# bjing2016/mdgen

Hardware: AMD Instinct MI355X
Metric: sampled MD frames/sec (higher is better)
Workload: dtype bf16; 1 GPU; tetrapeptide_fwdsim_crop4_T1000_B16; batch_per_gpu=16, num_frames=1000, crop=4, euler_steps=49, hipgraph=True, parallelism=batch-sharded x1, no collective

## Files before the change

### mdgen_amd/csrc/k_flash.hip

```cpp
#include "kernels.h"
#include "panel.h"
#include <type_traits>

namespace mdg {

__device__ __forceinline__ bf16x8 frag16(const unsigned char* p) { return *reinterpret_cast<const bf16x8*>(p); }

__device__ __forceinline__ bf16x8 frag8(const unsigned char* p) {
    const u32x2 v = *reinterpret_cast<const u32x2*>(p);
    const u32x4 w = u32x4{v[0], v[1], 0u, 0u};
    return __builtin_bit_cast(bf16x8, w);
}

struct KTile {
    u32x4 k0;
    u32x4 k1;
};
__device__ __forceinline__ void k_consts(KTile& t) {
    t.k1 = u32x4{0u, 0u, 0x3f803f80u, 0u};
    asm volatile("" : "+v"(t.k1));
}
struct VTile {
    u32x4 v0;
    u32x4 v1;
// ... 60 lines not shown
    float e[16];
#pragma unroll
    for (int j = 0; j < 16; ++j) e[j] = __builtin_amdgcn_exp2f(s[j]);
#pragma unroll
    for (int j = 0; j < 4; ++j) {
        pc.p0[j] = pack_bf16(e[2 * j], e[2 * j + 1]);
        pc.p1[j] = pack_bf16(e[8 + 2 * j], e[9 + 2 * j]);
    }
#pragma unroll
    for (int g = 0; g < 4; ++g) {
        __builtin_amdgcn_sched_group_barrier(0x008, 1, 0);
        __builtin_amdgcn_sched_group_barrier(0x402, 6, 0);
    }
    asm volatile("" : "+v"(pc.p0), "+v"(pc.p1) : "v"(k0), "v"(k1), "v"(qn.q0), "v"(qn.q1));
}

constexpr float kDefer = 8.f;

__device__ __forceinline__ void softmax_stats(Half& st, f32x16& s, QTile& q, uint32_t vm, int hh) {
    if (vm != 0xffffffffu) mask_scores(s, vm, hh);
    float t = fmaxf(s[0], s[1]);
#pragma unroll
    for (int r = 2; r < 16; r += 2) t = fmaxf(fmaxf(t, s[r]), s[r + 1]);
    t = half_max(t);
    if ((__builtin_amdgcn_ballot_w64(t > kDefer) | st.unanch) != 0) {
        const bool fin = t > -1e29f;
        const bool un = (st.unanch >> lane_id()) & 1ull;
        const bool mv = (t > kDefer) | (un & fin & (t < -kDefer));
        st.unanch &= ~__builtin_amdgcn_ballot_w64(fin);
        const float r = set_shift(q, mv ? st.m + t : st.m, hh);
        const float e = r - st.m;
        st.m = r;
        const float a = __builtin_amdgcn_exp2f(fminf(-e, 0.f));
#pragma unroll
        for (int i = 0; i < 16; ++i) {
            st.o[i] *= a;
            s[i] -= e;
        }
    }
}

#ifdef MDGEN_DEV_FLASH_STAMPS
__device__ unsigned long long g_flash_stamps[32768 * 16];
extern "C" int mdgen_dev_flash_stamps(void* host, size_t bytes) {
    return (int)hipMemcpyFromSymbol(host, HIP_SYMBOL(g_flash_stamps), bytes);
}
#define FLASH_STAMP(slot, v)                                                                          \
    if (lane == 0 && (long)blockIdx.x * 4 + w < 32768) g_flash_stamps[((long)blockIdx.x * 4 + w) * 16 + (slot)] = (v)
__device__ unsigned long long g_fproj_stamps[8192 * 16];
extern "C" int mdgen_dev_fproj_stamps(void* host, size_t bytes) {
    return (int)hipMemcpyFromSymbol(host, HIP_SYMBOL(g_fproj_stamps), bytes);
}
#define FPROJ_STAMP(slot, v)                                                                          \
    if (lane_id() == 0 && (long)blockIdx.x * 4 + w < 8192) g_fproj_stamps[((long)blockIdx.x * 4 + w) * 16 + (slot)] = (v)
#define FLASH_STAMP_ROW(w, hg) ((w) + 4096 * (hg))
#else
#define FLASH_STAMP(slot, v)
#define FPROJ_STAMP(slot, v)
#define FLASH_STAMP_ROW(w, hg) (w)
#endif

template <int N, class F>
__device__ __forceinline__ void static_for(F&& f) {
    if constexpr (N > 0) {
        static_for<N - 1>(f);
        f(std::integral_constant<int, N - 1>{});
    }
}

struct FlashStoreGlobal {
    __bf16* obuf;
    AxisMap ax;
    int seq, head;
    __device__ __forceinline__ void row(int, int pos, u32x2 a, u32x2 b, u32x2 c) const {
        u32x2* d = reinterpret_cast<u32x2*>(obuf + ax.token(seq, pos) * kC + head * kDH + (lane_id() >> 5) * 12);
        d[0] = a;
        d[1] = b;
        d[2] = c;
    }
    __device__ __forceinline__ void pad(int, int) const {}
};

template <int NQ>
struct FlashPre {
    QTile q[NQ];
    u32x4 kb0;
    u32x2 kb1;
    f32x4 bvl[3];
    u32x4 k0t0;
    u32x2 k0t1;
    uint32_t vmw;
};

__device__ __forceinline__ void* flash_uniform_ptr(const unsigned char* q_) {
    const unsigned long long a = (unsigned long long)q_;
    const unsigned lo = __builtin_amdgcn_readfirstlane((unsigned)a), hi = __builtin_amdgcn_readfirstlane((unsigned)(a >> 32));
    return (void*)(((unsigned long long)hi << 32) | lo);
}

template <int NQ>
__device__ __forceinline__ void flash_prefetch(const FlashParams p, const int seq, const int head, const int qc, FlashPre<NQ>& pre) {
    const int lane = lane_id(), hh = lane >> 5;
    const int len = p.ax.len, nt = p.ax.ntile();
    const long ftile = (long)(seq * kH + head) * nt;
    const unsigned char* qb = p.qf + ftile * kFragQ;
    const int qt0 = NQ * qc;
#pragma unroll
    for (int j = 0; j < NQ; ++j) {
        const int qt = (qt0 + j) * 32 < len ? qt0 + j : qt0;
        pre.q[j].q0 = frag16(qb + (long)qt * kFragQ + lane * 16);
        pre.q[j].q1 = frag8(qb + (long)qt * kFragQ + 1024 + lane * 8);
    }
    const bool bias_alone = (len & 31) == 0 && len >= 32;
    const unsigned char* kb = p.kf + (ftile + (bias_alone ? (len >> 5) : 0)) * kFragK;
    pre.kb0 = *reinterpret_cast<const u32x4*>(kb + hh * 32 * 16);
    pre.kb1 = *reinterpret_cast<const u32x2*>(kb + 1024 + hh * 32 * 8);
    const f32x4* bv = reinterpret_cast<const f32x4*>(p.bias_v + head * kDH + hh * 12);
    pre.bvl[0] = bv[0];
    pre.bvl[1] = bv[1];
    pre.bvl[2] = bv[2];
    const __amdgpu_buffer_rsrc_t krs = __builtin_amdgcn_make_buffer_rsrc(flash_uniform_ptr(p.kf + ftile * kFragK), 0, 0x7fffffff, 0x00020000);
    pre.k0t0 = __builtin_amdgcn_raw_buffer_load_b128(krs, lane * 16, 0, 0);
    pre.k0t1 = __builtin_amdgcn_raw_buffer_load_b64(krs, lane * 8 + 1024, 0, 0);
    pre.vmw = (p.vmask + (long)seq * p.vmask_stride)[lane];
}

template <int NQ, class Store>
__device__ __forceinline__ void flash_job(const FlashParams p, const int seq, const int head, const int qc, const int w,
                                          const FlashPre<NQ> pre, const Store store) {
    const int lane = lane_id(), hh = lane >> 5, ql = lane & 31;
    FLASH_STAMP(0, __builtin_amdgcn_s_memtime());
    FLASH_STAMP(4, __builtin_amdgcn_s_memrealtime());
    const int len = p.ax.len, nt = p.ax.ntile();
    const long ftile = (long)(seq * kH + head) * nt;
    const int qt0 = NQ * qc;
    QTile q[NQ];
    bool qvalid[NQ];
#pragma unroll
    for (int j = 0; j < NQ; ++j) {
        qvalid[j] = (qt0 + j) * 32 < len;
        q[j] = pre.q[j];
    }
    const bool bias_alone = (len & 31) == 0 && len >= 32;
    const u32x4 kb0 = pre.kb0;
    const u32x2 kb1 = pre.kb1;
    const f32x4 bvl[3] = {pre.bvl[0], pre.bvl[1], pre.bvl[2]};

    const __amdgpu_buffer_rsrc_t krs = __builtin_amdgcn_make_buffer_rsrc(flash_uniform_ptr(p.kf + ftile * kFragK), 0, 0x7fffffff, 0x00020000);
    const __amdgpu_buffer_rsrc_t vrs = __builtin_amdgcn_make_buffer_rsrc(flash_uniform_ptr(p.vf + ftile * kFragV), 0, 0x7fffffff, 0x00020000);
    const int koff = lane * 16, koff1 = lane * 8 + 1024;
    const int voff = ql <= kDH ? hh * 400 + ql * 16 : (int)0x80000000;
    auto issue_k = [&](KTile& t, int kt) __attribute__((always_inline)) {
        t.k0 = __builtin_amdgcn_raw_buffer_load_b128(krs, koff, kt * kFragK, 0);
        const u32x2 r = __builtin_amdgcn_raw_buffer_load_b64(krs, koff1, kt * kFragK, 0);
        t.k1[0] = r[0];
        t.k1[1] = r[1];
    };
    auto issue_v = [&](VTile& t, int kt) __attribute__((always_inline)) {
        t.v0 = __builtin_amdgcn_raw_buffer_load_b128(vrs, voff, kt * kFragV, 0);
        t.v1 = __builtin_amdgcn_raw_buffer_load_b128(vrs, voff + 800, kt * kFragV, 0);
    };
    KTile k0t;
    k0t.k0 = pre.k0t0;
    k0t.k1 = u32x4{pre.k0t1[0], pre.k0t1[1], 0x3f803f80u, 0u};
    const uint32_t* vmrow = p.vmask + (long)seq * p.vmask_stride;
    uint32_t vmw = pre.vmw;

    Half h[NQ];
    f32x16 s[2];
    PTile pt[2];
    KTile kx, ky;
    VTile vx, vy;
    int rot = 0, nrun = 1;
    auto phys = [&](int i) __attribute__((always_inline)) {
        const int t = i + rot;
        return t >= nrun ? t - nrun : t;
    };
    auto tile = [&](auto robust, int ti, KTile& kc, KTile& kn, VTile& vc, VTile& vprev) __attribute__((always_inline)) {
        constexpr bool kRobust = decltype(robust)::value;
        const int t = kRobust ? ti : phys(ti);
        const uint32_t vm = __builtin_amdgcn_readlane(vmw, t & 63);
        static_for<NQ>([&](auto J) __attribute__((always_inline)) {
            constexpr int j = decltype(J)::value;
            if constexpr (kRobust) softmax_stats(h[j], s[j & 1], q[j], vm, hh);
            else if (vm != 0xffffffffu) mask_scores(s[j & 1], vm, hh);
            __builtin_amdgcn_sched_barrier(0);
            if constexpr (j == 0) block(kc, q[1], s[1], vprev, pt[(NQ - 1) & 1], h[NQ - 1].o, s[0], pt[0]);
            else if constexpr (j < NQ - 1) block(kc, q[j + 1], s[(j + 1) & 1], vc, pt[(j - 1) & 1], h[j - 1].o, s[j & 1], pt[j & 1]);
            else block(kn, q[0], s[0], vc, pt[(j - 1) & 1], h[j - 1].o, s[j & 1], pt[j & 1]);
            __builtin_amdgcn_sched_barrier(0);
            if constexpr (j == 0) issue_v(vprev, kRobust ? ti + 1 : phys(ti + 1));
            if constexpr (j == NQ - 2) issue_k(kc, kRobust ? ti + 2 : phys(ti + 2));
            if constexpr (j == 0 || j == NQ - 2) __builtin_amdgcn_sched_barrier(0);
        });
    };
    auto run = [&](auto robust, const int nt, const int rot_) __attribute__((always_inline)) {
        rot = rot_;
        nrun = nt;
#pragma unroll
        for (int j = 0; j < NQ; ++j)
#pragma unroll
            for (int r = 0; r < 16; ++r) h[j].o[r] = opaque_zero();
        pt[(NQ - 1) & 1].p0 = pt[(NQ - 1) & 1].p1 = u32x4{0u, 0u, 0u, 0u};
        if (nt > 64) vmw = vmrow[lane];
        k_consts(kx);
        k_consts(ky);
        issue_k(kx, phys(0));
        issue_v(vy, phys(0));
        issue_k(ky, phys(1));
        issue_v(vx, phys(0));
        __builtin_amdgcn_sched_barrier(0);
        s[0] = scores(kx, q[0]);
        int t = 0;
        for (; t + 1 < nt; t += 2) {
            if ((t & 63) == 0 && t) vmw = vmrow[t + lane];
            tile(robust, t, kx, ky, vx, vy);
            tile(robust, t + 1, ky, kx, vy, vx);
        }
        const bf16x8 lp0 = __builtin_bit_cast(bf16x8, pt[(NQ - 1) & 1].p0), lp1 = __builtin_bit_cast(bf16x8, pt[(NQ - 1) & 1].p1);
        if (t < nt) {
            if ((t & 63) == 0 && t) vmw = vmrow[t + lane];
            tile(robust, t, kx, ky, vx, vy);
            h[NQ - 1].o = __builtin_amdgcn_mfma_f32_32x32x16_bf16(__builtin_bit_cast(bf16x8, vx.v0), __builtin_bit_cast(bf16x8, pt[(NQ - 1) & 1].p0), h[NQ - 1].o, 0, 0, 0);
            h[NQ - 1].o = __builtin_amdgcn_mfma_f32_32x32x16_bf16(__builtin_bit_cast(bf16x8, vx.v1), __builtin_bit_cast(bf16x8, pt[(NQ - 1) & 1].p1), h[NQ - 1].o, 0, 0, 0);
        } else {
            h[NQ - 1].o = __builtin_amdgcn_mfma_f32_32x32x16_bf16(__builtin_bit_cast(bf16x8, vy.v0), lp0, h[NQ - 1].o, 0, 0, 0);
            h[NQ - 1].o = __builtin_amdgcn_mfma_f32_32x32x16_bf16(__builtin_bit_cast(bf16x8, vy.v1), lp1, h[NQ - 1].o, 0, 0, 0);
        }
    };

    if (nt <= 64 && !p.force_robust) {
        const uint32_t want = lane == (len >> 5) ? 1u << (len & 31) : 0u;
        const bool only_bias = __builtin_amdgcn_ballot_w64(lane < nt && vmw != want) == 0;
        if (only_bias) {
            const f32x4 b0 = bvl[0], b1 = bvl[1], b2 = bvl[2];
            const u32x2 d0 = {pack_bf16(b0[0], b0[1]), pack_bf16(b0[2], b0[3])}, d1 = {pack_bf16(b1[0], b1[1]), pack_bf16(b1[2], b1[3])},
                        d2 = {pack_bf16(b2[0], b2[1]), pack_bf16(b2[2], b2[3])};
#pragma unroll
            for (int j = 0; j < NQ; ++j) {
                const int pos = (qt0 + j) * 32 + ql;
                if (qvalid[j] && pos < len) store.row(j, pos, d0, d1, d2);
                else store.pad(j, pos);
            }
            return;
        }
    }
    const int nt_fast = bias_alone ? nt - 1 : nt;
    float sbias[NQ], vbias[12];
    if (bias_alone) {
        const f32x4 b0 = bvl[0], b1 = bvl[1], b2 = bvl[2];
#pragma unroll
        for (int i = 0; i < 4; ++i) {
            vbias[i] = round_bf16(b0[i]);
            vbias[4 + i] = round_bf16(b1[i]);
            vbias[8 + i] = round_bf16(b2[i]);
        }
#pragma unroll
        for (int j = 0; j < NQ; ++j) {
            const u32x4 qa = __builtin_bit_cast(u32x4, q[j].q0);
            const u32x4 qb_ = __builtin_bit_cast(u32x4, q[j].q1);
            float d = 0.f;
#pragma unroll
            for (int i = 0; i < 4; ++i) d += bf16_lo(qa[i]) * bf16_lo(kb0[i]) + bf16_hi(qa[i]) * bf16_hi(kb0[i]);
#pragma unroll
            for (int i = 0; i < 2; ++i) d += bf16_lo(qb_[i]) * bf16_lo(kb1[i]) + bf16_hi(qb_[i]) * bf16_hi(kb1[i]);
            sbias[j] = d + __shfl_xor(d, 32, 64);
        }
    }
    bool robust_needed = p.force_robust != 0;
    {
        const uint32_t vm0 = __builtin_amdgcn_readlane(vmw, 0);
#pragma unroll
        for (int j = 0; j < NQ; ++j) {
            f32x16 s0 = scores(k0t, q[j]);
            if (vm0 != 0xffffffffu) mask_scores(s0, vm0, hh);
            float t0 = fmaxf(s0[0], s0[1]);
#pragma unroll
            for (int r = 2; r < 16; r += 2) t0 = fmaxf(fmaxf(t0, s0[r]), s0[r + 1]);
            t0 = half_max(t0);
            robust_needed |= __builtin_amdgcn_ballot_w64(!(t0 > -1e29f)) != 0;
            h[j].m = set_shift(q[j], t0 + kAnchor, hh);
        }
    }
    FLASH_STAMP(1, __builtin_amdgcn_s_memtime());
    FLASH_STAMP(6, (unsigned long long)robust_needed);
    FLASH_STAMP(8, (unsigned long long)__float_as_uint(h[0].m));
    if (!robust_needed) {
        run(std::false_type{}, nt_fast, (p.rotate && nt_fast > 2 && nt <= 64) ? (qc * nt_fast) / ((len + 32 * NQ - 1) / (32 * NQ)) : 0);
        if (bias_alone) {
#pragma unroll
            for (int j = 0; j < NQ; ++j) {
                const float pb = __builtin_amdgcn_exp2f(sbias[j] - h[j].m);
#pragma unroll
                for (int r = 0; r < 12; ++r) h[j].o[r] += pb * vbias[r];
                if (hh == 0) h[j].o[12] += pb;
            }
        }
        FLASH_STAMP(2, __builtin_amdgcn_s_memtime());
        bool bad = false;
#pragma unroll
        for (int j = 0; j < NQ; ++j) {
            const uint32_t lj = __float_as_uint(h[j].o[12]);
            bad |= (lj & 0x7f800000u) == 0x7f800000u;
            bad |= hh == 0 && (lj & 0x7f800000u) == 0u;
#pragma unroll
            for (int i = 0; i < 16; ++i) bad |= (__float_as_uint(h[j].o[i]) & 0x7f800000u) == 0x7f800000u;
        }
        FLASH_STAMP(9, (unsigned long long)__builtin_amdgcn_ballot_w64(bad));
        robust_needed = __builtin_amdgcn_ballot_w64(bad) != 0;
    }
    if (robust_needed) {
#pragma unroll
        for (int j = 0; j < NQ; ++j) {
            h[j].m = 0.f;
            h[j].unanch = ~0ull;
            set_shift(q[j], 0.f, hh);
        }
        run(std::true_type{}, nt, 0);
    }
    FLASH_STAMP(3, __builtin_amdgcn_s_memtime());
    FLASH_STAMP(11, (unsigned long long)__float_as_uint(h[0].m));
#ifdef MDGEN_DEV_FLASH_STAMPS
    if (lane == 0 && (long)blockIdx.x * 4 + w < 32768) g_flash_stamps[((long)blockIdx.x * 4 + w) * 16 + 6] |= (unsigned long long)robust_needed << 1;
#endif
#pragma unroll
    for (int j = 0; j < NQ; ++j) {
        const float l = __shfl(h[j].o[12], ql, 64);
        const int pos = (qt0 + j) * 32 + ql;
        if (qvalid[j] && pos < len) {
            const float inv = 1.0f / l;
            const f32x16 o = h[j].o;
            store.row(j, pos, u32x2{pack_bf16(o[0] * inv, o[1] * inv), pack_bf16(o[2] * inv, o[3] * inv)},
                      u32x2{pack_bf16(o[4] * inv, o[5] * inv), pack_bf16(o[6] * inv, o[7] * inv)},
                      u32x2{pack_bf16(o[8] * inv, o[9] * inv), pack_bf16(o[10] * inv, o[11] * inv)});
        } else {
            store.pad(j, pos);
        }
    }
    FLASH_STAMP(5, __builtin_amdgcn_s_memrealtime());
}

template <int NQ>
__global__ __launch_bounds__(256, NQ == 2 ? 3 : 2) void k_flash(const FlashParams p) {
    const int w = __builtin_amdgcn_readfirstlane(wave_id());
    const int nqc = (p.ax.len + 32 * NQ - 1) / (32 * NQ);
    const int xcd = blockIdx.x & 7, rest = blockIdx.x >> 3;
    const int qc = rest % nqc, pair = (rest / nqc) * 8 + xcd;
    const int seq = pair >> 2, hg = pair & 3;
    if (seq >= p.ax.nseq) return;
    const int head = hg * 4 + w;
    FlashPre<NQ> pre;
    flash_prefetch<NQ>(p, seq, head, qc, pre);
    flash_job<NQ>(p, seq, head, qc, w, pre, FlashStoreGlobal{p.obuf, p.ax, seq, head});
}

typedef __attribute__((address_space(3))) unsigned char lds_byte;
struct FlashStorePanel {
    lds_byte* panel;
    int head;
    __device__ __forceinline__ void put(int j, u32x2 a, u32x2 b, u32x2 c) const {
        const int lane = lane_id(), row = 32 * j + (lane & 31), byte = head * 48 + (lane >> 5) * 24;
        typedef __attribute__((address_space(3))) u32x2 lds_u32x2;
        *reinterpret_cast<lds_u32x2*>(panel + panel_off(row, byte, kC * 2)) = a;
        *reinterpret_cast<lds_u32x2*>(panel + panel_off(row, byte + 8, kC * 2)) = b;
        *reinterpret_cast<lds_u32x2*>(panel + panel_off(row, byte + 16, kC * 2)) = c;
    }
    __device__ __forceinline__ void row(int j, int, u32x2 a, u32x2 b, u32x2 c) const { put(j, a, b, c); }
    __device__ __forceinline__ void pad(int j, int) const { put(j, u32x2{0u, 0u}, u32x2{0u, 0u}, u32x2{0u, 0u}); }
};

__global__ __launch_bounds__(256, 2) void k_flash_proj(const FlashProjParams p) {
    constexpr int NQ = 2;
    static_assert(32 * NQ == kPanel, "one workgroup = one 64-row panel");
    __shared__ __attribute__((aligned(16))) unsigned char smem[sizeof(PanelRows) + kPanel * kC * 2];
// ... 105 lines not shown
```

### mdgen_amd/csrc/k_gemm.hip

```cpp
#include "kernels.h"
#include "panel.h"

namespace mdg {

constexpr int kRowB = kC * 2;
constexpr int kPanelBytes = kPanel * kRowB;

constexpr int kRopeLds = kRopeRow + 4;
constexpr int kBiasUnits = 3 * kC / 4;
struct QkvStage {
    float bias[3][kC];
    float rope[kPanel][kRopeLds];
};
struct Attn4Stage {
    float bias[3][kC];
    uint32_t tab[2][kL4Tab];
    float rope[4][kRopeLds];
};
__device__ __forceinline__ const f32x4* stage_bias_src(const QkvParams& p, int u) {
    const float* b = u < kC / 4 ? p.bq : u < 2 * (kC / 4) ? p.bk : p.bv;
    return reinterpret_cast<const f32x4*>(b) + (u % (kC / 4));
}
template <int NT>
struct QkvStager {
    static constexpr int kUnits = kBiasUnits + kPanel * 8, kPer = (kUnits + NT - 1) / NT;
    f32x4 r[kPer];
    __device__ __forceinline__ void load(const QkvParams& p, int pos0, int len, int tid) {
#pragma unroll
        for (int i = 0; i < kPer; ++i) {
            int u = tid + i * NT;
            if (u >= kUnits) u = kUnits - 1;
            const int v = u >= kBiasUnits ? u - kBiasUnits : 0;
            int pos = pos0 + (v >> 3);
            if (pos > len) pos = len;
            const f32x4* rs = reinterpret_cast<const f32x4*>(p.rope + (long)pos * kRopeRow) + (v & 7);
            r[i] = *(u < kBiasUnits ? stage_bias_src(p, u) : rs);
        }
    }
    __device__ __forceinline__ void store(QkvStage* st, int tid) const {
#pragma unroll
        for (int i = 0; i < kPer; ++i) {
            const int u = tid + i * NT;
            if (u < kBiasUnits) {
                reinterpret_cast<f32x4*>(&st->bias[0][0])[u] = r[i];
            } else if (u < kUnits) {
                const int v = u - kBiasUnits;
                *reinterpret_cast<f32x4*>(&st->rope[v >> 3][4 * (v & 7)]) = r[i];
            }
        }
    }
};
struct Attn4Stager {
    static constexpr int kTab0 = kBiasUnits, kRope0 = kTab0 + 2 * kL4Tab / 4, kUnits = kRope0 + 4 * 8;
    static_assert(kUnits <= 512 && kBiasUnits > 256, "two units per thread, the first always a bias unit");
    f32x4 r[2];
    __device__ __forceinline__ void load(const QkvParams& p, int tid) {
        r[0] = *stage_bias_src(p, tid);
        int u = tid + 256;
        if (u >= kUnits) u = kUnits - 1;
        const f32x4* src = u < kTab0    ? stage_bias_src(p, u < kTab0 ? u : 0)
                           : u < kRope0 ? reinterpret_cast<const f32x4*>(p.l4tab) + (u - kTab0)
                                        : reinterpret_cast<const f32x4*>(p.rope) + (u - kRope0);
        r[1] = *src;
    }
    __device__ __forceinline__ void store(Attn4Stage* st, int tid) const {
        reinterpret_cast<f32x4*>(&st->bias[0][0])[tid] = r[0];
        const int u = tid + 256;
        if (u < kTab0) {
            reinterpret_cast<f32x4*>(&st->bias[0][0])[u] = r[1];
        } else if (u < kRope0) {
            reinterpret_cast<f32x4*>(&st->tab[0][0])[u - kTab0] = r[1];
        } else if (u < kUnits) {
            const int v = u - kRope0;
            *reinterpret_cast<f32x4*>(&st->rope[v >> 3][4 * (v & 7)]) = r[1];
        }
    }
};

template <bool X1S>
__device__ __forceinline__ void rotate_pair(float x1, float x2, float c, float sn, float& e0, float& e1);
enum RopeForm { kRopeFree, kRopeX2C, kRopeHead0X1S };
template <bool ROPE, int TT = 2, bool STAGED = false, RopeForm RF = kRopeFree>
__device__ __forceinline__ void epilogue_heads_T(const f32x16* acc , const PanelRows* pr, int w,
                                                 const float* bias_perm, const float* rope,
                                                 bool small, int pos0, int len, int seq, int ntile, int tile0,
                                                 unsigned char* __restrict__ frag, __bf16* __restrict__ small_dst,
                                                 int which) {
    const int lane = lane_id(), hh = lane >> 5, tk = lane & 31;
    f32x4 bq[4][3];
    {
        const f32x4* bp = reinterpret_cast<const f32x4*>(bias_perm + (w * 2 + hh) * 48);
#pragma unroll
        for (int hd = 0; hd < 4; ++hd)
#pragma unroll
            for (int c = 0; c < 3; ++c) bq[hd][c] = bp[hd * 3 + c];
    }
    int tokv[TT], posv[TT];
    f32x4 rq[TT][4];
#pragma unroll
    for (int tt = 0; tt < TT; ++tt) {
        const int row = tt * 32 + tk;
        tokv[tt] = pr->tok[row];
        int pos = small ? (tokv[tt] >= 0 ? tokv[tt] % len : 0) : pos0 + row;
        if (pos > len) pos = len;
        posv[tt] = pos;
        if (ROPE) {
            const f32x4* rc = reinterpret_cast<const f32x4*>(STAGED ? rope + row * kRopeLds + 16 * hh : rope + (long)pos * kRopeRow + 16 * hh);
#pragma unroll
            for (int i = 0; i < 4; ++i) rq[tt][i] = rc[i];
        }
    }
#pragma unroll
    for (int tt = 0; tt < TT; ++tt) {
        const int token = tokv[tt];
        const bool valid = token >= 0;
        float cs[6], sn[6];
        if (ROPE) {
#pragma unroll
            for (int p = 0; p < 6; ++p) {
                cs[p] = rq[tt][p >> 2][p & 3];
                sn[p] = rq[tt][2 + (p >> 2)][p & 3];
            }
        }
        const int tile = tile0 + tt;
#pragma unroll
        for (int hd = 0; hd < 4; ++hd) {
            float e[12];
#pragma unroll
            for (int c = 0; c < 3; ++c) {
                const int ap = 3 * hd + c, ft = ap >> 2, a = ap & 3;
#pragma unroll
                for (int b = 0; b < 4; ++b) e[4 * c + b] = acc[ft * TT + tt][4 * a + b] + bq[hd][c][b];
            }
            if (ROPE) {
#pragma unroll
                for (int p = 0; p < 6; ++p) {
                    const float x1 = e[2 * p], x2 = e[2 * p + 1];
                    if (RF == kRopeFree) {
                        e[2 * p] = x1 * cs[p] - x2 * sn[p];
                        e[2 * p + 1] = x2 * cs[p] + x1 * sn[p];
                    } else if (RF == kRopeHead0X1S && hd == 0) {
                        rotate_pair<false>(x1, x2, cs[p], sn[p], e[2 * p], e[2 * p + 1]);
                    } else {
                        rotate_pair<true>(x1, x2, cs[p], sn[p], e[2 * p], e[2 * p + 1]);
                    }
                }
            }
            uint32_t u[6];
#pragma unroll
            for (int i = 0; i < 6; ++i) u[i] = pack_bf16(e[2 * i], e[2 * i + 1]);
            const int head = 4 * w + hd;
            if (small) {
                if (valid) {
                    u32x2* d = reinterpret_cast<u32x2*>(small_dst + (long)token * (3 * kC) + which * kC + head * kDH + hh * 12);
                    d[0] = u32x2{u[0], u[1]};
                    d[1] = u32x2{u[2], u[3]};
                    d[2] = u32x2{u[4], u[5]};
                }
            } else if (tile < ntile) {
                if (which == 1) {
                    unsigned char* base = frag + ((long)(seq * kH + head) * ntile + tile) * kFragK;
                    *reinterpret_cast<u32x4*>(base + lane * 16) = u32x4{u[0], u[1], u[2], u[3]};
                    *reinterpret_cast<u32x2*>(base + 1024 + lane * 8) = u32x2{u[4], u[5]};
                } else {
                    unsigned char* base = frag + ((long)(seq * kH + head) * ntile + tile) * kFragQ;
                    *reinterpret_cast<u32x4*>(base + lane * 16) = u32x4{u[0], u[1], u[2], u[3]};
                    *reinterpret_cast<u32x2*>(base + 1024 + lane * 8) = u32x2{u[4], u[5]};
                }
            }
        }
    }
}

template <int TT = 2>
__device__ __forceinline__ void epilogue_v_flash(const f32x16* acc , int w,
                                                 const float* bias_perm, int seq, int ntile, int tile0,
                                                 unsigned char* __restrict__ vf) {
    const int lane = lane_id(), hh = lane >> 5, n = lane & 31;
#pragma unroll
    for (int j = 0; j < 3; ++j) {
        const int col = 32 * j + n;
        const int hd = col / kDH, d = col - hd * kDH;
        const float b = bias_perm[w * 96 + col];
        const int head = 4 * w + hd;
#pragma unroll
        for (int tt = 0; tt < TT; ++tt) {
            const int tile = tile0 + tt;
            if (tile < ntile) {
                unsigned char* base = vf + ((long)(seq * kH + head) * ntile + tile) * kFragV + hh * 400 + d * 16;
                const f32x16 a = acc[tt * 3 + j];
                *reinterpret_cast<u32x4*>(base) = u32x4{pack_bf16(a[0] + b, a[1] + b), pack_bf16(a[2] + b, a[3] + b),
                                                         pack_bf16(a[4] + b, a[5] + b), pack_bf16(a[6] + b, a[7] + b)};
                *reinterpret_cast<u32x4*>(base + 800) =
                    u32x4{pack_bf16(a[8] + b, a[9] + b), pack_bf16(a[10] + b, a[11] + b),
                          pack_bf16(a[12] + b, a[13] + b), pack_bf16(a[14] + b, a[15] + b)};
            }
        }
    }
    if (lane < 32) {
        const int hd = lane & 3, tt = (lane >> 2) & 1, h2 = (lane >> 3) & 1, ks = lane >> 4;
        const int tile = tile0 + tt;
        if (tt < TT && tile < ntile)
            *reinterpret_cast<u32x4*>(vf + ((long)(seq * kH + 4 * w + hd) * ntile + tile) * kFragV + ks * 800 + h2 * 400 + kDH * 16) =
                u32x4{0x3f803f80u, 0x3f803f80u, 0x3f803f80u, 0x3f803f80u};
    }
}

__device__ __forceinline__ void write_bias_slots(const QkvParams& p, int seq, int w, bool do_k = true, bool do_v = true, int tpp = 2) {
    const int lane = lane_id();
    const int len = p.ax.len, nt = p.ax.ntile();
    const int kt = len >> 5, sl = len & 31;
    if (kt >= tpp * p.panels_per_seq) {
#pragma unroll
        for (int hd = 0; hd < 4; ++hd) {
            const long ft = (long)(seq * kH + 4 * w + hd) * nt + kt;
            unsigned char* kd = p.kf + ft * kFragK;
            u32x4* vd = reinterpret_cast<u32x4*>(p.vf + ft * kFragV);
            const u32x4 z = {0u, 0u, 0u, 0u}, ones = {0x3f803f80u, 0x3f803f80u, 0x3f803f80u, 0x3f803f80u};
            if (do_k) {
                *reinterpret_cast<u32x4*>(kd + lane * 16) = z;
                *reinterpret_cast<u32x2*>(kd + 1024 + lane * 8) = u32x2{0u, 0u};
            }
            const int r0 = lane, r1 = 64 + lane;
            if (do_v) {
                vd[r0] = (r0 % 25) == kDH ? ones : z;
                if (r1 < 100) vd[r1] = (r1 % 25) == kDH ? ones : z;
            }
        }
        __builtin_amdgcn_sched_barrier(0);
    }
    if (do_k && lane < 8) {
        const int hd = lane & 3, hh = lane >> 2, head = 4 * w + hd;
        const float* bk = p.bias_k + head * kDH;
        const float* rc = p.rope + (long)len * kRopeRow + 16 * hh;
        float e[12];
#pragma unroll
        for (int pp = 0; pp < 6; ++pp) {
            const int i = 6 * hh + pp;
            const float x1 = bk[i], x2 = bk[i + 12], c = rc[pp], sn = rc[8 + pp];
            e[2 * pp] = x1 * c - x2 * sn;
            e[2 * pp + 1] = x2 * c + x1 * sn;
        }
        unsigned char* base = p.kf + ((long)(seq * kH + head) * nt + kt) * kFragK;
        *reinterpret_cast<u32x4*>(base + (hh * 32 + sl) * 16) =
            u32x4{pack_bf16(e[0], e[1]), pack_bf16(e[2], e[3]), pack_bf16(e[4], e[5]), pack_bf16(e[6], e[7])};
        *reinterpret_cast<u32x2*>(base + 1024 + (hh * 32 + sl) * 8) = u32x2{pack_bf16(e[8], e[9]), pack_bf16(e[10], e[11])};
    }
    if (do_v && lane < kDH) {
        const int d = lane;
        const int dpsi = 12 * ((d >> 2) & 1) + 4 * (d >> 3) + (d & 3);
        const int hk = (sl >> 2) & 1, r = (sl & 3) + 4 * (sl >> 3);
#pragma unroll
        for (int hd = 0; hd < 4; ++hd) {
            const int head = 4 * w + hd;
            unsigned char* base = p.vf + ((long)(seq * kH + head) * nt + kt) * kFragV;
            const uint32_t v = pack_bf16(p.bias_v[head * kDH + dpsi], 0.f);
            *reinterpret_cast<uint16_t*>(base + (r >> 3) * 800 + hk * 400 + d * 16 + (r & 7) * 2) = (uint16_t)v;
        }
    }
}

#ifdef MDGEN_DEV_QKV_STAMPS
__device__ unsigned long long g_qkv_stamps[16384 * 8];
extern "C" int mdgen_dev_qkv_stamps(void* host, size_t bytes) {
    return (int)hipMemcpyFromSymbol(host, HIP_SYMBOL(g_qkv_stamps), bytes);
}
#define QKV_STAMP(slot)                                                                                      \
    if (!SMALL && lane_id() == 0 && (long)blockIdx.x * 4 + wave_id() < 16384)                                  \
    g_qkv_stamps[((long)blockIdx.x * 4 + wave_id()) * 8 + (slot)] = __builtin_amdgcn_s_memtime()
__device__ unsigned long long g_attn4_stamps[8192 * 16];
extern "C" int mdgen_dev_attn4_stamps(void* host, size_t bytes) {
    return (int)hipMemcpyFromSymbol(host, HIP_SYMBOL(g_attn4_stamps), bytes);
}
#define ATTN4_STAMP_DECL unsigned long long a4st[11] = {}
#define ATTN4_STAMP(slot)                          \
    a4st[slot] = __builtin_amdgcn_s_memtime();     \
    __builtin_amdgcn_sched_barrier(0)
#define ATTN4_STAMP_FLUSH                                                                                   \
    if (lane_id() == 0 && (long)blockIdx.x * 4 + wave_id() < 8192) {                                          \
        _Pragma("unroll") for (int k = 0; k < 11; ++k)                                                        \
            g_attn4_stamps[((long)blockIdx.x * 4 + wave_id()) * 16 + k] = a4st[k];                            \
    }
#else
#define QKV_STAMP(slot)
#define ATTN4_STAMP_DECL
#define ATTN4_STAMP(slot)
#define ATTN4_STAMP_FLUSH
#endif

template <bool SMALL, bool PRE = false>
__global__ __launch_bounds__(256, 2) void k_ln_qkv(const QkvParams p) {
    __shared__ __attribute__((aligned(16))) unsigned char smem[sizeof(PanelRows) + kPanelBytes];
    __shared__ __attribute__((aligned(16))) unsigned char stage_[SMALL ? 16 : sizeof(QkvStage)];
    QkvStage* const stage = reinterpret_cast<QkvStage*>(stage_);
    QkvStager<256> stager;
    PanelRows* pr = reinterpret_cast<PanelRows*>(smem);
    unsigned char* panel = smem + sizeof(PanelRows);
    int seq = 0, pos0 = 0, tile0 = 0;
    if (SMALL) {
        setup_rows_linear(pr, (long)blockIdx.x * kPanel, p.nrows, p.mm);
    } else {
        seq = blockIdx.x / p.panels_per_seq;
        const int pn = blockIdx.x - seq * p.panels_per_seq;
        pos0 = pn * kPanel;
        tile0 = pn * 2;
        stager.load(p, pos0, p.ax.len, threadIdx.x);
        setup_rows_axis(pr, p.ax, seq, pos0, p.mm);
        if (wave_id() == 0) {
            const int lane = lane_id(), len = p.ax.len, pos = pos0 + lane;
            const float mv = p.mk.at(p.ax.token(seq, pos < len ? pos : len - 1));
            const unsigned long long bal = __ballot(pos == len || (pos < len && mv != 0.f));
            uint32_t* vm = p.vmask + (long)seq * p.vmask_stride;
            if (lane < 2) vm[tile0 + lane] = (uint32_t)(bal >> (32 * lane));
            if (pn == p.panels_per_seq - 1) {
                const int idx = tile0 + 2 + lane;
                if (idx < p.vmask_stride) vm[idx] = idx == (len >> 5) ? 1u << (len & 31) : 0u;
                if (idx + 64 < p.vmask_stride) vm[idx + 64] = 0u;
            }
        }
    }
    QKV_STAMP(0);
    __syncthreads();
    if (!SMALL) stager.store(stage, threadIdx.x);
    const int w = __builtin_amdgcn_readfirstlane(wave_id()), lane = lane_id();
    const float *sbq = SMALL ? p.bq : stage->bias[0], *sbk = SMALL ? p.bk : stage->bias[1], *sbv = SMALL ? p.bv : stage->bias[2];
    const float* srope = SMALL ? p.rope : &stage->rope[0][0];
    f32x16 acc[6];
    if (PRE) {
        prologue_bf16<kC>(panel, pr, p.obuf);
        __syncthreads();
        wave_gemm<2, 3, 24, false, 4, true>(panel, kRowB, 0, 0, p.wo + (size_t)(3 * w) * 24 * 64 + lane, 24 * 64, acc);
        __syncthreads();
        epilogue_gate_residual_lds<3>(acc, pr, reinterpret_cast<float*>(panel) + w * (32 * 96), 96 * w, p.bo, p.mm, p.gate_chunk,
                                      true, p.h_rw);
        __syncthreads();
    }
    prologue_ln<false>(panel, pr, PRE ? p.h_rw : p.h, p.mm, p.shift_chunk, p.scale_chunk, 1e-6f);
    __syncthreads();
    QKV_STAMP(1);
    const int ntile = p.ax.ntile();
    const int len = p.ax.len;
    wave_gemm<2, 3, 24, true, 4, true>(panel, kRowB, 0, 0, p.wq + (size_t)(3 * w) * 24 * 64 + lane, 24 * 64, acc);
    QKV_STAMP(2);
    epilogue_heads_T<true, 2, !SMALL, SMALL ? kRopeFree : kRopeX2C>(acc, pr, w, sbq, srope, SMALL, pos0, len, seq, ntile, tile0, p.qf, p.qkv_small, 0);
    __builtin_amdgcn_sched_barrier(0);
    QKV_STAMP(3);
    wave_gemm<2, 3, 24, true, 4, true>(panel, kRowB, 0, 0, p.wk + (size_t)(3 * w) * 24 * 64 + lane, 24 * 64, acc);
    QKV_STAMP(4);
    epilogue_heads_T<true, 2, !SMALL, SMALL ? kRopeFree : kRopeX2C>(acc, pr, w, sbk, srope, SMALL, pos0, len, seq, ntile, tile0, p.kf, p.qkv_small, 1);
    __builtin_amdgcn_sched_barrier(0);
    QKV_STAMP(5);
    if (SMALL) {
        wave_gemm<2, 3, 24, true, 4, true>(panel, kRowB, 0, 0, p.wv + (size_t)(3 * w) * 24 * 64 + lane, 24 * 64, acc);
        epilogue_heads_T<false>(acc, pr, w, p.bv, nullptr, true, pos0, len, seq, ntile, tile0, nullptr, p.qkv_small, 2);
    } else {
        wave_gemm<2, 3, 24, false, 4, true>(panel, kRowB, 0, 0, p.wv + (size_t)(3 * w) * 24 * 64 + lane, 24 * 64, acc);
        QKV_STAMP(6);
        epilogue_v_flash(acc, w, sbv, seq, ntile, tile0, p.vf);
        if ((int)blockIdx.x - seq * p.panels_per_seq == p.panels_per_seq - 1) {
            __builtin_amdgcn_sched_barrier(0);
            write_bias_slots(p, seq, w);
        }
        QKV_STAMP(7);
    }
}

template <int J>
__device__ __forceinline__ float quad_bcast(float v) {
    return __builtin_bit_cast(float, __builtin_amdgcn_update_dpp(0, __builtin_bit_cast(int, v), J * 0x55, 0xf, 0xf, true));
}
template <int J>
__device__ __forceinline__ float fmac_dpp(float acc, float k, float q) {
    asm("v_fmac_f32_dpp %0, %1, %2 quad_perm:[%3,%3,%3,%3] row_mask:0xf bank_mask:0xf bound_ctrl:1" : "+v"(acc) : "v"(k), "v"(q), "n"(J));
    return acc;
}
template <int J>
__device__ __forceinline__ float mul_dpp(float k, float q) {
    float r;
    asm("v_mul_f32_dpp %0, %1, %2 quad_perm:[%3,%3,%3,%3] row_mask:0xf bank_mask:0xf bound_ctrl:1" : "=v"(r) : "v"(k), "v"(q), "n"(J));
    return r;
}
__device__ __forceinline__ void dpp_fence(float (&k)[12]) {
    asm volatile("s_nop 1"
                 : "+v"(k[0]), "+v"(k[1]), "+v"(k[2]), "+v"(k[3]), "+v"(k[4]), "+v"(k[5]), "+v"(k[6]), "+v"(k[7]), "+v"(k[8]), "+v"(k[9]),
                   "+v"(k[10]), "+v"(k[11]));
}
__device__ __forceinline__ float half_sum(float x) {
    const auto r = __builtin_amdgcn_permlane32_swap(__float_as_uint(x), __float_as_uint(x), false, false);
    return __uint_as_float(r[0]) + __uint_as_float(r[1]);
}
template <int TT = 2>
__device__ __forceinline__ void head_values(const f32x16* acc, int tt, int hd, const f32x4 (&bq)[3], float (&e)[12]) {
#pragma unroll
    for (int c = 0; c < 3; ++c) {
        const int ap = 3 * hd + c, ft = ap >> 2, a = ap & 3;
#pragma unroll
        for (int b = 0; b < 4; ++b) e[4 * c + b] = acc[ft * TT + tt][4 * a + b] + bq[c][b];
    }
}
template <bool X1S>
__device__ __forceinline__ void rotate_pair(float x1, float x2, float c, float sn, float& e0, float& e1) {
    const float a = x2 * sn;
    e0 = __builtin_fmaf(x1, c, -a);
    if (X1S) {
        const float b = x1 * sn;
        e1 = __builtin_fmaf(x2, c, b);
    } else {
        const float b = x2 * c;
        e1 = __builtin_fmaf(x1, sn, b);
    }
}
__device__ __forceinline__ void load_head_bias(const float* bias_perm, int w, int hh, f32x4 (&bq)[4][3]) {
    const f32x4* bp = reinterpret_cast<const f32x4*>(bias_perm + (w * 2 + hh) * 48);
#pragma unroll
    for (int hd = 0; hd < 4; ++hd)
#pragma unroll
        for (int c = 0; c < 3; ++c) bq[hd][c] = bp[hd * 3 + c];
}


template <bool SPLIT, bool HALF = false>
__global__ __launch_bounds__(512, 1) void k_ln_qkv8(const QkvParams p) {
    static_assert(!HALF || SPLIT, "32-row workgroups exist in the split form only");
    constexpr int TT = HALF ? 1 : 2, kRows = 32 * TT;
    __shared__ __attribute__((aligned(16))) unsigned char smem[sizeof(PanelRows) + kPanelBytes];
    __shared__ __attribute__((aligned(16))) QkvStage stage;
    QkvStager<512> stager;
    PanelRows* pr = reinterpret_cast<PanelRows*>(smem);
    unsigned char* panel = smem + sizeof(PanelRows);
    const int blk = SPLIT ? blockIdx.x >> 1 : blockIdx.x, half = SPLIT ? blockIdx.x & 1 : 0;
    const int seq = blk / p.panels_per_seq;
    const int pn = blk - seq * p.panels_per_seq;
    const int pos0 = pn * kRows, tile0 = pn * TT;
    stager.load(p, pos0, p.ax.len, threadIdx.x);
    setup_rows_axis(pr, p.ax, seq, pos0, p.mm, kRows);
    if (wave_id() == 0 && half == 0) {
        const int lane = lane_id(), len = p.ax.len, pos = pos0 + lane;
        const float mv = p.mk.at(p.ax.token(seq, pos < len ? pos : len - 1));
        const unsigned long long bal = __ballot(pos == len || (pos < len && mv != 0.f));
        uint32_t* vm = p.vmask + (long)seq * p.vmask_stride;
        if (lane < TT) vm[tile0 + lane] = (uint32_t)(bal >> (32 * lane));
        if (pn == p.panels_per_seq - 1) {
            const int idx = tile0 + TT + lane;
            if (idx < p.vmask_stride) vm[idx] = idx == (len >> 5) ? 1u << (len & 31) : 0u;
            if (idx + 64 < p.vmask_stride) vm[idx + 64] = 0u;
        }
    }
    __syncthreads();
    stager.store(&stage, threadIdx.x);
    const int w8 = __builtin_amdgcn_readfirstlane(wave_id()), g = w8 >> 2, w = w8 & 3, lane = lane_id();
    if (HALF) {
        if (g == 0) prologue_ln<false, 0, 1>(panel, pr, p.h, p.mm, p.shift_chunk, p.scale_chunk, 1e-6f, w, lane);
        else prologue_ln<false, 1, 2>(panel, pr, p.h, p.mm, p.shift_chunk, p.scale_chunk, 1e-6f, w, lane);
    } else {
        if (g == 0) prologue_ln<false, 0, 2>(panel, pr, p.h, p.mm, p.shift_chunk, p.scale_chunk, 1e-6f, w, lane);
        else prologue_ln<false, 2, 4>(panel, pr, p.h, p.mm, p.shift_chunk, p.scale_chunk, 1e-6f, w, lane);
    }
    __syncthreads();
    const int ntile = p.ax.ntile(), len = p.ax.len;
    const bool last = pn == p.panels_per_seq - 1;
    f32x16 acc[3 * TT];
    const bool do_q = SPLIT ? half == 0 && g == 0 : g == 0, do_k = SPLIT ? half == 0 && g == 1 : g == 0;
    const bool do_v = SPLIT ? half == 1 && g == 0 : g == 1;
    if (do_q) {
        wave_gemm<TT, 3, 24, true, 4, true>(panel, kRowB, 0, 0, p.wq + (size_t)(3 * w) * 24 * 64 + lane, 24 * 64, acc);
        epilogue_heads_T<true, TT, true, HALF ? kRopeHead0X1S : kRopeX2C>(acc, pr, w, stage.bias[0], &stage.rope[0][0], false, pos0, len, seq, ntile, tile0, p.qf, p.qkv_small, 0);
        __builtin_amdgcn_sched_barrier(0);
    }
    if (do_k) {
        wave_gemm<TT, 3, 24, true, 4, true>(panel, kRowB, 0, 0, p.wk + (size_t)(3 * w) * 24 * 64 + lane, 24 * 64, acc);
        epilogue_heads_T<true, TT, true, HALF ? kRopeHead0X1S : kRopeX2C>(acc, pr, w, stage.bias[1], &stage.rope[0][0], false, pos0, len, seq, ntile, tile0, p.kf, p.qkv_small, 1);
        if (last) {
            __builtin_amdgcn_sched_barrier(0);
            write_bias_slots(p, seq, w, true, false, TT);
        }
    }
    if (do_v) {
        wave_gemm<TT, 3, 24, false, 4, true>(panel, kRowB, 0, 0, p.wv + (size_t)(3 * w) * 24 * 64 + lane, 24 * 64, acc);
        epilogue_v_flash<TT>(acc, w, stage.bias[2], seq, ntile, tile0, p.vf);
        if (last) {
            __builtin_amdgcn_sched_barrier(0);
            write_bias_slots(p, seq, w, false, true, TT);
        }
    }
}

constexpr int kAttn4KPF = 2, kAttn4VPF = 3;
template <bool PROJ, bool HALF = false>
__global__ __launch_bounds__(256, 2) void k_ln_qkv_attn4(const QkvParams p) {
    static_assert(!HALF || PROJ, "the half-panel form is the whole sub-layer");
    constexpr int TT = HALF ? 1 : 2, kRows = HALF ? 32 : kPanel;
    __shared__ __attribute__((aligned(16))) unsigned char smem[sizeof(PanelRows) + kPanelBytes];
    __shared__ uint32_t qstash[HALF ? 1 : 4][24][64];
    __shared__ __attribute__((aligned(16))) Attn4Stage stage;
    Attn4Stager stager;
    PanelRows* pr = reinterpret_cast<PanelRows*>(smem);
    unsigned char* panel = smem + sizeof(PanelRows);
    ATTN4_STAMP_DECL;
    ATTN4_STAMP(0);
    stager.load(p, threadIdx.x);
    {
        const long row0 = (long)blockIdx.x * kRows, rend = row0 + kRows;
        setup_rows_linear(pr, row0, rend < p.nrows ? rend : p.nrows, p.mm);
    }
    __syncthreads();
    stager.store(&stage, threadIdx.x);
    const int w = __builtin_amdgcn_readfirstlane(wave_id());
    constexpr int t0 = 0;
    if (HALF) prologue_ln<false, 0, 2>(panel, pr, p.h, p.mm, p.shift_chunk, p.scale_chunk, 1e-6f, w, lane_id());
    else prologue_ln<false>(panel, pr, p.h, p.mm, p.shift_chunk, p.scale_chunk, 1e-6f);
    __syncthreads();
    ATTN4_STAMP(1);
    const int lane = lane_id(), hh = lane >> 5, tk = lane & 31;
    constexpr int L = 4;
    int tok[TT];
    float mval[TT];
#pragma unroll
    for (int tt = 0; tt < TT; ++tt) {
        tok[tt] = pr->tok[(t0 + tt) * 32 + tk];
        mval[tt] = p.mk.at(tok[tt] < 0 ? 0 : tok[tt]);
    }
    auto load_rope = [&](f32x4 (&rq)[TT][4]) {
#pragma unroll
        for (int tt = 0; tt < TT; ++tt) {
            const int tc = tok[tt] < 0 ? 0 : tok[tt];
            const f32x4* rc = reinterpret_cast<const f32x4*>(&stage.rope[tc & (L - 1)][16 * hh]);
#pragma unroll
            for (int i = 0; i < 4; ++i) rq[tt][i] = rc[i];
        }
    };
    f32x16 acc[3 * TT];
    f32x4 bb[4][3];
    f32x4 rq[TT][4];
    wave_gemm<TT, 3, 24, true, 4, true>(panel, kRowB, t0, 0, p.wq + (size_t)(3 * w) * 24 * 64 + lane, 24 * 64, acc);
    ATTN4_STAMP(2);
    load_head_bias(stage.bias[0], w, hh, bb);
    load_rope(rq);
    uint32_t qp[TT][4][6];
#pragma unroll
    for (int tt = 0; tt < TT; ++tt)
#pragma unroll
        for (int hd = 0; hd < 4; ++hd) {
            float e[12];
            head_values<TT>(acc, tt, hd, bb[hd], e);
#pragma unroll
            for (int q = 0; q < 6; ++q) {
                const float c = rq[tt][q >> 2][q & 3], sn = rq[tt][2 + (q >> 2)][q & 3];
                float r0, r1;
                rotate_pair<HALF>(e[2 * q], e[2 * q + 1], c, sn, r0, r1);
                qp[tt][hd][q] = pack_bf16(r0, r1);
            }
        }
    if constexpr (!HALF) {
#pragma unroll
        for (int hd = 0; hd < 4; ++hd)
#pragma unroll
            for (int q = 0; q < 6; ++q) qstash[w][hd * 6 + q][lane] = qp[TT - 1][hd][q];
    }
    ATTN4_STAMP(3);
    __builtin_amdgcn_sched_barrier(0);
    wave_gemm<TT, 3, 24, true, HALF ? 4 : kAttn4KPF, true>(panel, kRowB, t0, 0, p.wk + (size_t)(3 * w) * 24 * 64 + lane, 24 * 64, acc);
    ATTN4_STAMP(4);
    load_head_bias(stage.bias[1], w, hh, bb);
    load_rope(rq);
#pragma unroll
    for (int tt = 0; tt < TT; ++tt)
#pragma unroll
        for (int hd = 0; hd < 4; ++hd) {
            float k[12];
            head_values<TT>(acc, tt, hd, bb[hd], k);
#pragma unroll
            for (int c = 0; c < 3; ++c) {
                const int ap = 3 * hd + c, ft = ap >> 2, a = ap & 3;
#pragma unroll
                for (int b2 = 0; b2 < 2; ++b2) {
                    const int q = 2 * c + b2;
                    const float cs = rq[tt][q >> 2][q & 3], sn = rq[tt][2 + (q >> 2)][q & 3];
                    float r0, r1;
                    rotate_pair<HALF>(k[2 * q], k[2 * q + 1], cs, sn, r0, r1);
                    acc[ft * TT + tt][4 * a + 2 * b2] = r0;
                    acc[ft * TT + tt][4 * a + 2 * b2 + 1] = r1;
                }
            }
        }
    ATTN4_STAMP(5);
    __builtin_amdgcn_sched_barrier(0);
    float P[TT][4][5];
    {
#pragma unroll
        for (int hd = 0; hd < 4; ++hd) {
            const uint32_t* kt = &stage.tab[0][((2 * w + hh) * 4 + hd) * 6];
            float kb[12];
#pragma unroll
            for (int q = 0; q < 6; ++q) {
                kb[2 * q] = bf16_lo(kt[q]);
                kb[2 * q + 1] = bf16_hi(kt[q]);
            }
#pragma unroll
            for (int tt = 0; tt < TT; ++tt) {
                float k[12], qf[12];
#pragma unroll
                for (int c = 0; c < 3; ++c) {
                    const int ap = 3 * hd + c, ft = ap >> 2, a = ap & 3;
#pragma unroll
                    for (int b2 = 0; b2 < 4; ++b2) k[4 * c + b2] = acc[ft * TT + tt][4 * a + b2];
                }
#pragma unroll
                for (int q = 0; q < 6; ++q) {
                    const uint32_t u = (HALF || tt == 0) ? qp[tt][hd][q] : qstash[w][hd * 6 + q][lane];
                    qf[2 * q] = bf16_lo(u);
                    qf[2 * q + 1] = bf16_hi(u);
                }
                dpp_fence(k);
                float s[5];
                s[0] = mul_dpp<0>(k[0], qf[0]);
                s[1] = mul_dpp<1>(k[0], qf[0]);
                s[2] = mul_dpp<2>(k[0], qf[0]);
                s[3] = mul_dpp<3>(k[0], qf[0]);
                s[4] = 0.f;
#pragma unroll
                for (int i = 0; i < 12; ++i) {
                    if (i > 0) {
                        s[0] = fmac_dpp<0>(s[0], k[i], qf[i]);
                        s[1] = fmac_dpp<1>(s[1], k[i], qf[i]);
                        s[2] = fmac_dpp<2>(s[2], k[i], qf[i]);
                        s[3] = fmac_dpp<3>(s[3], k[i], qf[i]);
                    }
                    s[4] += qf[i] * kb[i];
                }
#pragma unroll
                for (int j = 0; j < 5; ++j) s[j] = half_sum(s[j]);
                const float m0 = quad_bcast<0>(mval[tt]), m1 = quad_bcast<1>(mval[tt]), m2 = quad_bcast<2>(mval[tt]),
// ... 772 lines not shown
```

Before: 127,800 frames/s.

## Bake key-validity masking into V fragments instead of masking scores in flash loop

Padded or masked key rows are now zeroed in the V fragments and their ones-column when the QKV epilogue writes them. The padding K tile is filled with copies of the bias key row, so masked keys no longer contribute to the output or the softmax denominator. This lets the fast flash path drop the per-tile readlane and mask_scores work and the vmask reloads, keeping masking only in the robust path. The trade is extra bitmask work in the producer epilogue and a stronger reliance on the zeroed-V numerics being correct, for example with large scores.

```diff
diff --git a/mdgen_amd/csrc/k_flash.hip b/mdgen_amd/csrc/k_flash.hip
--- a/mdgen_amd/csrc/k_flash.hip
+++ b/mdgen_amd/csrc/k_flash.hip
@@ -236,6 +236,7 @@
     const int voff = ql <= kDH ? hh * 400 + ql * 16 : (int)0x80000000;
     auto issue_k = [&](KTile& t, int kt) __attribute__((always_inline)) {
         t.k0 = __builtin_amdgcn_raw_buffer_load_b128(krs, koff, kt * kFragK, 0);
+        asm volatile("" : "+v"(t.k1));
         const u32x2 r = __builtin_amdgcn_raw_buffer_load_b64(krs, koff1, kt * kFragK, 0);
         t.k1[0] = r[0];
         t.k1[1] = r[1];
@@ -262,12 +263,11 @@
     };
     auto tile = [&](auto robust, int ti, KTile& kc, KTile& kn, VTile& vc, VTile& vprev) __attribute__((always_inline)) {
         constexpr bool kRobust = decltype(robust)::value;
-        const int t = kRobust ? ti : phys(ti);
-        const uint32_t vm = __builtin_amdgcn_readlane(vmw, t & 63);
+        uint32_t vm = 0xffffffffu;
+        if constexpr (kRobust) vm = __builtin_amdgcn_readlane(vmw, ti & 63);
         static_for<NQ>([&](auto J) __attribute__((always_inline)) {
             constexpr int j = decltype(J)::value;
             if constexpr (kRobust) softmax_stats(h[j], s[j & 1], q[j], vm, hh);
-            else if (vm != 0xffffffffu) mask_scores(s[j & 1], vm, hh);
             __builtin_amdgcn_sched_barrier(0);
             if constexpr (j == 0) block(kc, q[1], s[1], vprev, pt[(NQ - 1) & 1], h[NQ - 1].o, s[0], pt[0]);
             else if constexpr (j < NQ - 1) block(kc, q[j + 1], s[(j + 1) & 1], vc, pt[(j - 1) & 1], h[j - 1].o, s[j & 1], pt[j & 1]);
@@ -279,6 +279,7 @@
         });
     };
     auto run = [&](auto robust, const int nt, const int rot_) __attribute__((always_inline)) {
+        constexpr bool kRobust = decltype(robust)::value;
         rot = rot_;
         nrun = nt;
 #pragma unroll
@@ -286,7 +287,7 @@
 #pragma unroll
             for (int r = 0; r < 16; ++r) h[j].o[r] = opaque_zero();
         pt[(NQ - 1) & 1].p0 = pt[(NQ - 1) & 1].p1 = u32x4{0u, 0u, 0u, 0u};
-        if (nt > 64) vmw = vmrow[lane];
+        if constexpr (kRobust) vmw = vmrow[lane];
         k_consts(kx);
         k_consts(ky);
         issue_k(kx, phys(0));
@@ -297,13 +298,13 @@
         s[0] = scores(kx, q[0]);
         int t = 0;
         for (; t + 1 < nt; t += 2) {
-            if ((t & 63) == 0 && t) vmw = vmrow[t + lane];
+            if (kRobust && (t & 63) == 0 && t) vmw = vmrow[t + lane];
             tile(robust, t, kx, ky, vx, vy);
             tile(robust, t + 1, ky, kx, vy, vx);
         }
         const bf16x8 lp0 = __builtin_bit_cast(bf16x8, pt[(NQ - 1) & 1].p0), lp1 = __builtin_bit_cast(bf16x8, pt[(NQ - 1) & 1].p1);
         if (t < nt) {
-            if ((t & 63) == 0 && t) vmw = vmrow[t + lane];
+            if (kRobust && (t & 63) == 0 && t) vmw = vmrow[t + lane];
             tile(robust, t, kx, ky, vx, vy);
             h[NQ - 1].o = __builtin_amdgcn_mfma_f32_32x32x16_bf16(__builtin_bit_cast(bf16x8, vx.v0), __builtin_bit_cast(bf16x8, pt[(NQ - 1) & 1].p0), h[NQ - 1].o, 0, 0, 0);
             h[NQ - 1].o = __builtin_amdgcn_mfma_f32_32x32x16_bf16(__builtin_bit_cast(bf16x8, vx.v1), __builtin_bit_cast(bf16x8, pt[(NQ - 1) & 1].p1), h[NQ - 1].o, 0, 0, 0);
diff --git a/mdgen_amd/csrc/k_gemm.hip b/mdgen_amd/csrc/k_gemm.hip
--- a/mdgen_amd/csrc/k_gemm.hip
+++ b/mdgen_amd/csrc/k_gemm.hip
@@ -172,11 +172,29 @@
     }
 }
 
+__device__ __forceinline__ unsigned long long panel_key_validity(const QkvParams& p, int seq, int pos0) {
+    const int len = p.ax.len, pos = pos0 + lane_id();
+    const float mv = p.mk.at(p.ax.token(seq, pos < len ? pos : len - 1));
+    return __ballot(pos == len || (pos < len && mv != 0.f));
+}
+__device__ __forceinline__ void v_valid_dwords(uint32_t vm, int hk, uint32_t (&m)[8]) {
+    const uint32_t vmh = vm >> (4 * hk);
+#pragma unroll
+    for (int j = 0; j < 8; ++j) {
+        const int r0 = 2 * j, r1 = 2 * j + 1;
+        const uint32_t lo = (vmh >> ((r0 & 3) + 8 * (r0 >> 2))) & 1u, hi = (vmh >> ((r1 & 3) + 8 * (r1 >> 2))) & 1u;
+        m[j] = ((0u - lo) & 0x0000ffffu) | ((0u - hi) & 0xffff0000u);
+    }
+}
+
 template <int TT = 2>
 __device__ __forceinline__ void epilogue_v_flash(const f32x16* acc , int w,
                                                  const float* bias_perm, int seq, int ntile, int tile0,
-                                                 unsigned char* __restrict__ vf) {
+                                                 unsigned char* __restrict__ vf, unsigned long long valid) {
     const int lane = lane_id(), hh = lane >> 5, n = lane & 31;
+    uint32_t vm[TT];
+#pragma unroll
+    for (int tt = 0; tt < TT; ++tt) vm[tt] = __builtin_amdgcn_readfirstlane((uint32_t)(valid >> (32 * tt)));
 #pragma unroll
     for (int j = 0; j < 3; ++j) {
         const int col = 32 * j + n;
@@ -189,20 +207,38 @@
             if (tile < ntile) {
                 unsigned char* base = vf + ((long)(seq * kH + head) * ntile + tile) * kFragV + hh * 400 + d * 16;
                 const f32x16 a = acc[tt * 3 + j];
-                *reinterpret_cast<u32x4*>(base) = u32x4{pack_bf16(a[0] + b, a[1] + b), pack_bf16(a[2] + b, a[3] + b),
-                                                         pack_bf16(a[4] + b, a[5] + b), pack_bf16(a[6] + b, a[7] + b)};
-                *reinterpret_cast<u32x4*>(base + 800) =
-                    u32x4{pack_bf16(a[8] + b, a[9] + b), pack_bf16(a[10] + b, a[11] + b),
-                          pack_bf16(a[12] + b, a[13] + b), pack_bf16(a[14] + b, a[15] + b)};
+                u32x4 v0 = u32x4{pack_bf16(a[0] + b, a[1] + b), pack_bf16(a[2] + b, a[3] + b),
+                                 pack_bf16(a[4] + b, a[5] + b), pack_bf16(a[6] + b, a[7] + b)};
+                u32x4 v1 = u32x4{pack_bf16(a[8] + b, a[9] + b), pack_bf16(a[10] + b, a[11] + b),
+                                 pack_bf16(a[12] + b, a[13] + b), pack_bf16(a[14] + b, a[15] + b)};
+                if (vm[tt] != 0xffffffffu) {
+                    uint32_t m[8];
+                    v_valid_dwords(vm[tt], hh, m);
+#pragma unroll
+                    for (int i = 0; i < 4; ++i) {
+                        v0[i] &= m[i];
+                        v1[i] &= m[4 + i];
+                    }
+                }
+                *reinterpret_cast<u32x4*>(base) = v0;
+                *reinterpret_cast<u32x4*>(base + 800) = v1;
             }
         }
     }
     if (lane < 32) {
         const int hd = lane & 3, tt = (lane >> 2) & 1, h2 = (lane >> 3) & 1, ks = lane >> 4;
         const int tile = tile0 + tt;
-        if (tt < TT && tile < ntile)
-            *reinterpret_cast<u32x4*>(vf + ((long)(seq * kH + 4 * w + hd) * ntile + tile) * kFragV + ks * 800 + h2 * 400 + kDH * 16) =
-                u32x4{0x3f803f80u, 0x3f803f80u, 0x3f803f80u, 0x3f803f80u};
+        if (tt < TT && tile < ntile) {
+            u32x4 ones = u32x4{0x3f803f80u, 0x3f803f80u, 0x3f803f80u, 0x3f803f80u};
+            const uint32_t vml = tt == 0 ? vm[0] : vm[TT - 1];
+            if (vml != 0xffffffffu) {
+                uint32_t m[8];
+                v_valid_dwords(vml, h2, m);
+#pragma unroll
+                for (int i = 0; i < 4; ++i) ones[i] &= ks ? m[4 + i] : m[i];
+            }
+            *reinterpret_cast<u32x4*>(vf + ((long)(seq * kH + 4 * w + hd) * ntile + tile) * kFragV + ks * 800 + h2 * 400 + kDH * 16) = ones;
+        }
     }
 }
 
@@ -210,27 +246,20 @@
     const int lane = lane_id();
     const int len = p.ax.len, nt = p.ax.ntile();
     const int kt = len >> 5, sl = len & 31;
-    if (kt >= tpp * p.panels_per_seq) {
+    if (do_v && kt >= tpp * p.panels_per_seq) {
 #pragma unroll
         for (int hd = 0; hd < 4; ++hd) {
             const long ft = (long)(seq * kH + 4 * w + hd) * nt + kt;
-            unsigned char* kd = p.kf + ft * kFragK;
             u32x4* vd = reinterpret_cast<u32x4*>(p.vf + ft * kFragV);
-            const u32x4 z = {0u, 0u, 0u, 0u}, ones = {0x3f803f80u, 0x3f803f80u, 0x3f803f80u, 0x3f803f80u};
-            if (do_k) {
-                *reinterpret_cast<u32x4*>(kd + lane * 16) = z;
-                *reinterpret_cast<u32x2*>(kd + 1024 + lane * 8) = u32x2{0u, 0u};
-            }
+            const u32x4 z = {0u, 0u, 0u, 0u}, one0 = {0x00003f80u, 0u, 0u, 0u};
             const int r0 = lane, r1 = 64 + lane;
-            if (do_v) {
-                vd[r0] = (r0 % 25) == kDH ? ones : z;
-                if (r1 < 100) vd[r1] = (r1 % 25) == kDH ? ones : z;
-            }
+            vd[r0] = r0 == kDH ? one0 : z;
+            if (r1 < 100) vd[r1] = z;
         }
         __builtin_amdgcn_sched_barrier(0);
     }
-    if (do_k && lane < 8) {
-        const int hd = lane & 3, hh = lane >> 2, head = 4 * w + hd;
+    if (do_k) {
+        const int hd = lane & 3, hh = (lane >> 2) & 1, head = 4 * w + hd;
         const float* bk = p.bias_k + head * kDH;
         const float* rc = p.rope + (long)len * kRopeRow + 16 * hh;
         float e[12];
@@ -242,9 +271,16 @@
             e[2 * pp + 1] = x2 * c + x1 * sn;
         }
         unsigned char* base = p.kf + ((long)(seq * kH + head) * nt + kt) * kFragK;
-        *reinterpret_cast<u32x4*>(base + (hh * 32 + sl) * 16) =
-            u32x4{pack_bf16(e[0], e[1]), pack_bf16(e[2], e[3]), pack_bf16(e[4], e[5]), pack_bf16(e[6], e[7])};
-        *reinterpret_cast<u32x2*>(base + 1024 + (hh * 32 + sl) * 8) = u32x2{pack_bf16(e[8], e[9]), pack_bf16(e[10], e[11])};
+        const u32x4 k0 = u32x4{pack_bf16(e[0], e[1]), pack_bf16(e[2], e[3]), pack_bf16(e[4], e[5]), pack_bf16(e[6], e[7])};
+        const u32x2 k1 = u32x2{pack_bf16(e[8], e[9]), pack_bf16(e[10], e[11])};
+#pragma unroll
+        for (int i = 0; i < 4; ++i) {
+            const int s = sl + (lane >> 3) + 8 * i;
+            if (s < 32) {
+                *reinterpret_cast<u32x4*>(base + (hh * 32 + s) * 16) = k0;
+                *reinterpret_cast<u32x2*>(base + 1024 + (hh * 32 + s) * 8) = k1;
+            }
+        }
     }
     if (do_v && lane < kDH) {
         const int d = lane;
@@ -297,6 +333,7 @@
     PanelRows* pr = reinterpret_cast<PanelRows*>(smem);
     unsigned char* panel = smem + sizeof(PanelRows);
     int seq = 0, pos0 = 0, tile0 = 0;
+    unsigned long long valid = ~0ull;
     if (SMALL) {
         setup_rows_linear(pr, (long)blockIdx.x * kPanel, p.nrows, p.mm);
     } else {
@@ -306,10 +343,10 @@
         tile0 = pn * 2;
         stager.load(p, pos0, p.ax.len, threadIdx.x);
         setup_rows_axis(pr, p.ax, seq, pos0, p.mm);
+        valid = panel_key_validity(p, seq, pos0);
         if (wave_id() == 0) {
-            const int lane = lane_id(), len = p.ax.len, pos = pos0 + lane;
-            const float mv = p.mk.at(p.ax.token(seq, pos < len ? pos : len - 1));
-            const unsigned long long bal = __ballot(pos == len || (pos < len && mv != 0.f));
+            const int lane = lane_id(), len = p.ax.len;
+            const unsigned long long bal = valid;
             uint32_t* vm = p.vmask + (long)seq * p.vmask_stride;
             if (lane < 2) vm[tile0 + lane] = (uint32_t)(bal >> (32 * lane));
             if (pn == p.panels_per_seq - 1) {
@@ -356,7 +393,7 @@
     } else {
         wave_gemm<2, 3, 24, false, 4, true>(panel, kRowB, 0, 0, p.wv + (size_t)(3 * w) * 24 * 64 + lane, 24 * 64, acc);
         QKV_STAMP(6);
-        epilogue_v_flash(acc, w, sbv, seq, ntile, tile0, p.vf);
+        epilogue_v_flash(acc, w, sbv, seq, ntile, tile0, p.vf, valid);
         if ((int)blockIdx.x - seq * p.panels_per_seq == p.panels_per_seq - 1) {
             __builtin_amdgcn_sched_barrier(0);
             write_bias_slots(p, seq, w);
@@ -434,10 +471,10 @@
     const int pos0 = pn * kRows, tile0 = pn * TT;
     stager.load(p, pos0, p.ax.len, threadIdx.x);
     setup_rows_axis(pr, p.ax, seq, pos0, p.mm, kRows);
+    const unsigned long long valid = panel_key_validity(p, seq, pos0);
     if (wave_id() == 0 && half == 0) {
-        const int lane = lane_id(), len = p.ax.len, pos = pos0 + lane;
-        const float mv = p.mk.at(p.ax.token(seq, pos < len ? pos : len - 1));
-        const unsigned long long bal = __ballot(pos == len || (pos < len && mv != 0.f));
+        const int lane = lane_id(), len = p.ax.len;
+        const unsigned long long bal = valid;
         uint32_t* vm = p.vmask + (long)seq * p.vmask_stride;
         if (lane < TT) vm[tile0 + lane] = (uint32_t)(bal >> (32 * lane));
         if (pn == p.panels_per_seq - 1) {
@@ -477,7 +514,7 @@
     }
     if (do_v) {
         wave_gemm<TT, 3, 24, false, 4, true>(panel, kRowB, 0, 0, p.wv + (size_t)(3 * w) * 24 * 64 + lane, 24 * 64, acc);
-        epilogue_v_flash<TT>(acc, w, stage.bias[2], seq, ntile, tile0, p.vf);
+        epilogue_v_flash<TT>(acc, w, stage.bias[2], seq, ntile, tile0, p.vf, valid);
         if (last) {
             __builtin_amdgcn_sched_barrier(0);
             write_bias_slots(p, seq, w, false, true, TT);
```

Measured after the change: 133,600 frames/s (median of 6 runs). 4.6% higher.
